# JakobHavtorn/benchmarking-lvms

Hardware: AMD Instinct MI355X
Metric: audio frames/sec training (VRNN, 16 kHz mu-law) (higher is better)
Workload: dtype f32

## Files before the change

benchmarking-lvms_amd/csrc/core.hip:

```cpp
#include <stdarg.h>
#include <string.h>

#include <stdlib.h>

#include <mutex>

#include "common.h"

namespace blvm {

static thread_local char g_err[512] = "";

void set_error(const char* fmt, ...) {
  va_list ap;
  va_start(ap, fmt);
  vsnprintf(g_err, sizeof(g_err), fmt, ap);
  va_end(ap);
}

}

namespace blvm {
namespace {
struct I32Chunk { int32_t v[256]; };
__global__ __launch_bounds__(256) void upload_i32_kernel(I32Chunk c, int32_t* dst, int n) {
  if ((int)threadIdx.x < n) dst[threadIdx.x] = c.v[threadIdx.x];
}
}
}

extern "C" int blvm_upload_i32(const int32_t* host, int n, int32_t* dst, void* stream) {
  using namespace blvm;
  BLVM_REQUIRE(n >= 0 && (n == 0 || (host != nullptr && dst != nullptr)), "upload_i32: null pointer");
  for (int off = 0; off < n; off += 256) {
    I32Chunk c;
    const int m = n - off < 256 ? n - off : 256;
    memcpy(c.v, host + off, sizeof(int32_t) * m);
    hipLaunchKernelGGL(upload_i32_kernel, dim3(1), dim3(256), 0, static_cast<hipStream_t>(stream), c, dst + off, m);
  }
  BLVM_CHECK_LAUNCH("upload_i32");
  return BLVM_OK;
}

namespace blvm {
namespace {
struct PchainCtl {
  std::mutex mu;
  int device = -1;
  unsigned* dev = nullptr;
  unsigned* host = nullptr;
  unsigned* host_dev = nullptr;
  unsigned epoch = 0;
  unsigned taken = 0;
};
PchainCtl& pchain_ctl_state() {
  static PchainCtl c;
  return c;
}
}

namespace {
int g_pchain_max_b = -1, g_pchain_tune = -1;
unsigned long long* g_pchain_prof = nullptr;
}
unsigned long long* pchain_profile_buffer() { return g_pchain_prof; }
int pchain_max_batch() {
  if (g_pchain_max_b < 0) {
    const char* e = getenv("BLVM_PCHAIN");
    const char* m = getenv("BLVM_PCHAIN_MAX_B");
    g_pchain_max_b = (e && atoi(e) == 0) ? 0 : (m ? atoi(m) : 128);
    for (const char* v : {"HSA_CU_MASK", "ROC_GLOBAL_CU_MASK"})
      if (const char* cm = getenv(v); cm && *cm) g_pchain_max_b = 0;
  }
  return g_pchain_max_b;
}
static_assert(OP_F32 == BLVM_DTYPE_F32 && OP_BF16 == BLVM_DTYPE_BF16 && OP_F16 == BLVM_DTYPE_F16, "operand types are the ABI values");
static int g_operand_dtype = -1;
OpType operand_type() {
  if (g_operand_dtype < 0) {
    const char* e = getenv("BLVM_DTYPE");
    g_operand_dtype = !e ? OP_F32
                      : (strcmp(e, "bf16") == 0 || strcmp(e, "1") == 0) ? OP_BF16
                      : (strcmp(e, "f16") == 0 || strcmp(e, "2") == 0)  ? OP_F16
                                                                          : OP_F32;
  }
  return static_cast<OpType>(g_operand_dtype);
}
int pchain_tune() {
  if (g_pchain_tune < 0) {
    const char* e = getenv("BLVM_PCHAIN_TUNE");
    g_pchain_tune = e ? atoi(e) : 20;
  }
  return g_pchain_tune;
}

int pchain_ctl(unsigned** dev, unsigned** host_dev, unsigned* epoch) {
  PchainCtl& c = pchain_ctl_state();
  std::lock_guard<std::mutex> lock(c.mu);
  int d = 0;
  BLVM_HIP(hipGetDevice(&d));
  if (c.device != d) {
    BLVM_HIP(hipMalloc(reinterpret_cast<void**>(&c.dev), 64));
    BLVM_HIP(hipMemset(c.dev, 0, 64));
    BLVM_HIP(hipHostMalloc(reinterpret_cast<void**>(&c.host), 64, hipHostMallocMapped));
    memset(c.host, 0, 64);
    BLVM_HIP(hipHostGetDevicePointer(reinterpret_cast<void**>(&c.host_dev), c.host, 0));
    c.device = d;
    c.epoch = 0;
    c.taken = 0;
  }
  *dev = c.dev;
  *host_dev = c.host_dev;
  *epoch = ++c.epoch;
  if (c.epoch == 0) *epoch = ++c.epoch;
  return BLVM_OK;
}
}

extern "C" int blvm_pchain_configure(int max_batch, int waves) {
  if (waves > 0 && waves != 16) {
    blvm::set_error("blvm_pchain_configure: waves = %d; the persistent kernels run 16 waves per workgroup", waves);
    return BLVM_EINVAL;
  }
  if (max_batch >= 0) blvm::g_pchain_max_b = max_batch;
  return BLVM_OK;
}

extern "C" int blvm_set_operand_dtype(int dtype) {
  if (dtype != BLVM_DTYPE_F32 && dtype != BLVM_DTYPE_BF16 && dtype != BLVM_DTYPE_F16) {
    blvm::set_error("blvm_set_operand_dtype: %d is none of BLVM_DTYPE_F32 (0), BLVM_DTYPE_BF16 (1), BLVM_DTYPE_F16 (2)", dtype);
    return BLVM_EINVAL;
  }
  blvm::g_operand_dtype = dtype;
  return BLVM_OK;
}
extern "C" int blvm_get_operand_dtype(void) { return blvm::operand_type(); }

extern "C" int blvm_pchain_max_batch(void) { return std::min(blvm::pchain_max_batch(), 128); }

extern "C" int blvm_pchain_tune(int bits) {
  blvm::g_pchain_tune = bits;
  return BLVM_OK;
}

extern "C" int blvm_pchain_profile(unsigned long long* device_buffer) {
  blvm::g_pchain_prof = device_buffer;
  return BLVM_OK;
}

extern "C" int blvm_async_errors(unsigned* last_code) {
  blvm::PchainCtl& c = blvm::pchain_ctl_state();
  std::lock_guard<std::mutex> lock(c.mu);
  if (!c.host) return 0;
  const volatile unsigned* h = c.host;
  if (last_code) *last_code = h[1];
  return (int)h[0];
}

extern "C" int blvm_async_errors_take(unsigned* last_code) {
  blvm::PchainCtl& c = blvm::pchain_ctl_state();
  std::lock_guard<std::mutex> lock(c.mu);
  if (!c.host) return 0;
  const volatile unsigned* h = c.host;
  const unsigned total = h[0];
  const unsigned fresh = total - c.taken;
  c.taken = total;
  if (last_code) *last_code = fresh ? h[1] : 0u;
  return (int)fresh;
}

extern "C" int blvm_version(void) { return 130;  }

extern "C" const char* blvm_last_error(void) { return blvm::g_err; }

// ... 13 lines not shown
```

benchmarking-lvms_amd/csrc/vrnn_static.h:

```cpp
#pragma once
#include <algorithm>
#include <initializer_list>

#include "pchain.h"

namespace blvm {
namespace pchain {

struct LinkRange {
  int ct, wg0, nwg;
};
struct VrnnFwdDeal {
  int def_n, half, g;
  LinkRange hproj, prior, post, head, phi, gru;
};
inline VrnnFwdDeal vrnn_fwd_deal(int ctH, int ctZ, int ctR, int tl, int cus, bool shared) {
  VrnnFwdDeal d;
  d.def_n = shared ? 0 : range_for(3 * ctR * tl, std::min(cus / 4, 64));
  d.half = range_for(ctH * tl, (cus - d.def_n) / 2);
  d.g = 2 * d.half;
  const int wide = shared ? d.half : d.g;
  d.hproj = shared ? LinkRange{3 * ctR, d.half, d.half} : LinkRange{3 * ctR, d.g, d.def_n};
  d.prior = LinkRange{ctH, 0, d.half};
  d.post = LinkRange{ctH, d.half, d.half};
  d.head = LinkRange{ctZ, 0, range_for(ctZ * tl, wide)};
  d.phi = LinkRange{ctH, 0, range_for(ctH * tl, wide)};
  d.gru = LinkRange{ctR, 0, range_for(ctR * tl, d.g)};
  return d;
}
struct VrnnBwdDeal {
  int def_n, half, g, spare;
  bool split3;
  LinkRange grub, part[3], dphi, gb, wide_h, dz, prior, post;
};
inline VrnnBwdDeal vrnn_bwd_deal(int ctH, int ctZ, int ctR, int tl, int cus, bool shared, bool allow_split3) {
  VrnnBwdDeal d;
  d.def_n = shared ? 0 : range_for(ctR * tl, std::min(cus / 4, 64));
  d.half = range_for(ctH * tl, (cus - d.def_n) / 2);
  d.g = 2 * d.half;
  const int wide = shared ? d.half : d.g;
  d.spare = cus - d.g - d.def_n;
  d.split3 = !shared && d.spare >= 8 && d.half >= 8 && allow_split3;
  d.grub = LinkRange{ctR, 0, range_for(ctR * tl, d.g)};
  d.part[0] = LinkRange{ctH, 0, range_for(ctH * tl, d.half)};
  d.part[1] = LinkRange{ctH, d.half, range_for(ctH * tl, d.half)};
  d.part[2] = LinkRange{ctH, d.g + d.def_n, d.split3 ? range_for(ctH * tl, d.spare) : 0};
  d.dphi = LinkRange{ctH, 0, range_for(ctH * tl, wide)};
  d.gb = shared ? LinkRange{ctR, d.half, d.half} : LinkRange{ctR, d.g, d.def_n};
  d.wide_h = LinkRange{ctH, 0, range_for(ctH * tl, wide)};
  d.dz = LinkRange{ctZ, 0, range_for(ctZ * tl, wide)};
  d.prior = LinkRange{ctH, 0, d.half};
  d.post = LinkRange{ctH, d.half, d.half};
  return d;
}

constexpr std::initializer_list<int> kFwdResident = {1, 2, 3, 4, 5};
constexpr std::initializer_list<int> kBwdResident = {0, 1, 2, 3, 5, 6, 7, 8, 9};
inline bool one_tile_each(const Program& p, std::initializer_list<int> links) {
  for (int i : links)
    if (tiles_per_workgroup((p.B + 15) / 16, p.d[i].ct, p.d[i].nwg, p.xcd != 0) > 1) return false;
  return true;
}

}
}
```

benchmarking-lvms_amd/csrc/vrnn_static.hip:

```cpp
#include <algorithm>
#include <mutex>

#include "common.h"
#include "pchain.h"
#include "vrnn_static.h"

namespace blvm {
namespace {
using namespace pchain;

struct SPtr {
  float* base;
  int stride;
  __device__ __forceinline__ float* at(int s) const { return base + (long)s * stride; }
};

constexpr int kMaxTiles = 8;
__device__ __forceinline__ int tile_lanes(int w, int wg0, int nwg, int rt, int ct, bool xcd) {
  TileIter it(w, wg0, nwg, rt, ct, xcd);
  const int lane = threadIdx.x & 63;
  it.j += lane * it.step;
  return (lane < kMaxTiles && it.valid()) ? (it.r0() | (it.c() << 16)) : -1;
}
__device__ __forceinline__ int tile_count(int lanes) { return __popcll(__ballot(lanes >= 0)); }

constexpr int kAnatBase = 128, kAnatRole = 512, kAnatSlots = 48;
#ifdef PCHAIN_TPROF
__device__ __forceinline__ void anat_begin(unsigned* tab) {
  for (int i = threadIdx.x; i < kAnatSlots * 8; i += blockDim.x) tab[i] = 0u;
  __syncthreads();
}
__device__ __forceinline__ void anat_arm(Poll& pl) { pl.rpolls = 0; pl.t_st = 0; }
__device__ __forceinline__ void anat_note(unsigned* tab, int slot, const Poll& pl) {
  const unsigned long long now = wall_clock64();
  if ((threadIdx.x & 63) == 0 && pl.rpolls != 0) {
    unsigned* q = tab + (slot * 2 + (threadIdx.x < 256 ? 0 : 1)) * 4;
    atomicAdd(q, 1u); atomicAdd(q + 1, pl.rpolls); atomicAdd(q + 2, (unsigned)(pl.t_ok - pl.t_issue));
    atomicAdd(q + 3, (unsigned)((pl.t_st != 0 ? pl.t_st : now) - pl.t_ok));
  }
}
__device__ __forceinline__ void anat_end(const unsigned* tab, unsigned long long* prof, int role, bool chosen) {
  __syncthreads();
  if (prof != nullptr && chosen)
    for (int i = threadIdx.x; i < kAnatSlots * 8; i += blockDim.x) prof[kAnatBase + role * kAnatRole + i] = tab[i];
}
#define ANAT(x) x
#else
#define ANAT(x)
#endif

struct LinChainArgs {
  SPtr a16, orm, o16;
  const float *W, *bias;
  int ldo, n16, B, s0, S, wg0, nwg, ct, xcd;
  Ctl ctl;
  int pace_early, pace_epi;
  ANAT(unsigned long long* prof;)
};
template <class PC>
__device__ __forceinline__ PC chain_pace(const LinChainArgs& a) {
  if constexpr (PC::paced) return PC{a.pace_early, a.pace_epi};
  else return PC();
}

template <int NW, int K, bool RES, class PC = PaceOff>
__global__ __launch_bounds__(NW * 64, 1) void static_lin_chain_kernel(LinChainArgs a) {
  __shared__ __attribute__((aligned(16))) float red[2][NW * 256];
  ANAT(__shared__ unsigned anat[kAnatSlots * 8]; anat_begin(anat);)
  const int w = blockIdx.x, B = a.B;
  const int tiles = tile_lanes(w, a.wg0, a.nwg, (B + 15) / 16, a.ct, a.xcd != 0);
  const int nt = tile_count(tiles);
  if (nt == 0) return;
  Poll pl{a.ctl, 0u, false, 1};
  int par = 0;
  if constexpr (RES) {
    const int trc = __builtin_amdgcn_readlane(tiles, 0), r0 = trc & 0xffff, c0 = (trc >> 16) * 16;
    WRegs<OP_F32, 1, K / (16 * NW)> ws;
    const float* const Ws[1] = {a.W};
    const int cs[1] = {c0};
    load_w<NW, OP_F32, 1, K / (16 * NW)>(ws.w, Ws, cs, K);
    const PC pace = chain_pace<PC>(a);
    for (int s = a.s0; s < a.S; ++s) {
      pl.code = (unsigned)s << 4;
      auto late = [&]() { return LinLate{a.bias, nullptr, nullptr, 0, 0, false, true, 0.f, Out{a.orm.at(s), a.ldo, false, a.o16.at(s), a.n16}}; };
      ANAT(anat_arm(pl);)
      tile_lin_late<NW, OP_F32>(a.a16.at(s), 0, true, a.W, K, late, r0, c0, B, red[par], pl, nullptr, nullptr, 0, ws, pace);
      ANAT(anat_note(anat, 0, pl);)
      par ^= 1;
    }
    ANAT(anat_end(anat, a.prof, 0, w == a.wg0);)
    return;
  }
  for (int s = a.s0; s < a.S; ++s) {
    pl.code = (unsigned)s << 4;
    const float* A = a.a16.at(s);
    auto late = [&]() { return LinLate{a.bias, nullptr, nullptr, 0, 0, false, true, 0.f, Out{a.orm.at(s), a.ldo, false, a.o16.at(s), a.n16}}; };
    for (int tk = 0; tk < nt; ++tk) {
      const int trc = __builtin_amdgcn_readlane(tiles, tk);
      tile_lin_late<NW, false>(A, 0, true, a.W, K, late, trc & 0xffff, (trc >> 16) * 16, B, red[par], pl);
      par ^= 1;
    }
  }
}

constexpr int kH = 256, kR = 512;

struct LinArgs {
  SPtr a, a2, a3, add, gate, orm, o16, o16b;
  const float *W, *bias;
  int ld0, ld1, ld2, ld3, n16, n16b, w_width;
  float slope;
};
struct SeqArgs {
  SPtr a0, add0, aux[4], orm[4], o16[4];
  const float* W[4];
  int ld[4], ldadd0, ldgate, n16;
  float slope;
};
struct HeadArgs {
  SPtr P, Q, eps, mu_p, sd_p, mu_q, sd_q, raw_p, raw_q, muq_raw, z, z16, z16b;
  const float *Wp, *bp, *Wq, *bq;
  int ld3, n16, n16b, Z, residual;
  float beta, inv_beta, sd_eps;
};
struct GruArgs {
  SPtr X, xg, gh, hprev, hrm, h16, h16b, rg, ug, ng;
  const float *Wih, *bih;
  int ld0, ld3, n16, n16b, R;
};
struct DzArgs {
  SPtr D, add, mu_q, sd_q, mu_p, sd_p, eps, raw_q, raw_p, muq_raw, dqh, dqh16, dph, dph16;
  const float *WT, *c_raw, *c_fn;
  const int32_t* x_sl;
  int ld1, ld3, n16, Z, residual, stride, t0, first_gemm;
  float fn_floor, beta, sd_eps;
};
struct GrubArgs {
  SPtr D0, D1, g_in, rg, ug, ng, gh, hprev, dd, dgi, dgi16, dgh, dgh16, ga, g_add;
  const float *W0, *W1, *g_out;
  int ld0, ld1, ld3, n16, R, first_gemm, end_gates, first_gin;
};
struct Deal {
  int wg0, nwg, ct, s_begin, s_end, idx;
};

struct Walk {
  float* red0;
  float* red1;
  int par, B;
  Poll pl;
  ANAT(unsigned* anat;)
  __device__ __forceinline__ float* red() { par ^= 1; return par ? red0 : red1; }
  __device__ __forceinline__ void at(const Deal& d, int s, bool gentle, unsigned li = 0) {
// ... 95 lines not shown
    if (li == 0) tile_lin_late<NW, OP_F32>(A, 0, true, q.W[li], K0, late, tr0, tc0, wk.B, wk.red(), wk.pl, nullptr, nullptr, 0, rr.first, P0());
    else tile_lin_late<NW, OP_F32>(A, 0, true, q.W[li], K, late, tr0, tc0, wk.B, wk.red(), wk.pl, nullptr, nullptr, 0, rr.rest[li > 0 ? li - 1 : 0], Paced());
    ANAT(anat_note(wk.anat, 4 * d.idx + li, wk.pl);)
    A = q.o16[li].at(s);
  }
}

template <int NW, class PC = PaceOff>
__device__ __forceinline__ void visit_head(const HeadArgs& q, const Deal& d, int s, int tiles, int nt, Walk& wk, const Res<kH, 4>& ws) {
  if (nt == 0 || s < d.s_begin || s >= d.s_end) return;
  wk.at(d, s, false);
  const HeadOut o{q.mu_p.at(s), q.sd_p.at(s), q.mu_q.at(s), q.sd_q.at(s), q.raw_p.at(s), q.raw_q.at(s), q.muq_raw.at(s),
                  Out{q.z.at(s), q.ld3, false, q.z16.at(s), q.n16, q.z16b.at(s), q.n16b}};
  const int trc = __builtin_amdgcn_readlane(tiles, 0);
  ANAT(anat_arm(wk.pl);)
  tile_head<NW, OP_F32>(q.P.at(s), q.Q.at(s), true, q.Wp, q.bp, q.Wq, q.bq, q.eps.at(s), o, kH, q.Z, q.residual, q.beta, q.inv_beta, q.sd_eps,
                        trc & 0xffff, (trc >> 16) * 16, wk.B, wk.red(), wk.pl, ws, PC());
  ANAT(anat_note(wk.anat, 4 * d.idx, wk.pl);)
}

template <int NW, class PC = PaceOff>
__device__ __forceinline__ void visit_gru(const GruArgs& q, const Deal& d, int s, int tiles, int nt, Walk& wk, const Res<kH, 3>& ws) {
  if (nt == 0 || s < d.s_begin || s >= d.s_end) return;
  wk.at(d, s, false);
  const Out o{q.hrm.at(s), q.ld3, true, q.h16.at(s), q.n16, q.h16b.at(s), q.n16b};
  const int trc = __builtin_amdgcn_readlane(tiles, 0);
  ANAT(anat_arm(wk.pl);)
  tile_gru<NW, OP_F32>(q.X.at(s), 0, true, q.Wih, kH, q.xg.at(s), q.bih, q.gh.at(s), q.hprev.at(s), q.ld0, q.R, o, q.rg.at(s), q.ug.at(s), q.ng.at(s),
                       trc & 0xffff, (trc >> 16) * 16, wk.B, wk.red(), wk.pl, ws, PC());
  ANAT(anat_note(wk.anat, 4 * d.idx, wk.pl);)
}

template <int NW, class PC = PaceOff>
__device__ __forceinline__ void visit_dz(const DzArgs& q, const Deal& d, int s, int tiles, int nt, Walk& wk, const Res<kH>& ws) {
  if (nt == 0 || s < d.s_begin || s >= d.s_end) return;
  wk.at(d, s, false);
  DzIn z;
  z.mu_q = q.mu_q.at(s); z.sd_q = q.sd_q.at(s); z.mu_p = q.mu_p.at(s); z.sd_p = q.sd_p.at(s); z.eps = q.eps.at(s); z.raw_q = q.raw_q.at(s);
  z.raw_p = q.raw_p.at(s); z.muq_raw = q.muq_raw.at(s);
  z.x_sl = q.x_sl; z.c_raw = q.c_raw; z.c_fn = q.c_fn;
  z.t = q.t0 - s; z.stride = q.stride; z.residual = q.residual;
  z.fn_floor = q.fn_floor; z.beta = q.beta; z.sd_eps = q.sd_eps;
  z.has_gemm = s >= q.first_gemm;
  const Out oq{q.dqh.at(s), q.ld3, false, q.dqh16.at(s), q.n16}, op{q.dph.at(s), q.ld3, false, q.dph16.at(s), q.n16};
  const int trc = __builtin_amdgcn_readlane(tiles, 0);
  ANAT(anat_arm(wk.pl);)
  tile_dz<NW, OP_F32>(q.D.at(s), q.WT, nullptr, nullptr, true, q.add.at(s), q.ld1, false, z, oq, op, kH, q.Z, trc & 0xffff, (trc >> 16) * 16, wk.B,
                      wk.red(), wk.pl, ws, PC());
  ANAT(anat_note(wk.anat, 4 * d.idx, wk.pl);)
}

template <int NW, class PC = PaceOff>
__device__ __forceinline__ void visit_grub(const GrubArgs& q, const Deal& d, int s, int tiles, int nt, Walk& wk, const Res<kH, 2>& ws) {
  if (nt == 0 || s < d.s_begin || s >= d.s_end) return;
  wk.at(d, s, false);
  GrubIn g;
  g.D0 = q.D0.at(s); g.D1 = q.D1.at(s); g.W0 = q.W0; g.W1 = q.W1; g.g_in = q.g_in.at(s); g.g_add = q.g_add.at(s); g.ld_gadd = q.ld1;
  g.rg = q.rg.at(s); g.ug = q.ug.at(s); g.ng = q.ng.at(s); g.gh = q.gh.at(s); g.hprev = q.hprev.at(s); g.dd = q.dd.at(s); g.ldh = q.ld0;
  g.dgi = Out{q.dgi.at(s), q.ld3, false, q.dgi16.at(s), q.n16};
  g.dgh = Out{q.dgh.at(s), q.ld3, false, q.dgh16.at(s), q.n16};
  g.ga = q.ga.at(s); g.g_out = const_cast<float*>(q.g_out);
  g.has_gemm = s >= q.first_gemm; g.has_gates = s < q.end_gates; g.has_gin = s >= q.first_gin;
  const int trc = __builtin_amdgcn_readlane(tiles, 0);
  ANAT(anat_arm(wk.pl);)
  tile_grub<NW, OP_F32>(g, kH, q.R, trc & 0xffff, (trc >> 16) * 16, wk.B, wk.red(), wk.pl, ws, PC());
  ANAT(anat_note(wk.anat, 4 * d.idx, wk.pl);)
}

template <class A>
__device__ __forceinline__ const A& kargs() {
  typedef const __attribute__((address_space(4))) char kchar;
  kchar* p = (kchar*)__builtin_amdgcn_kernarg_segment_ptr();
  asm volatile("" : "+s"(p));
  return *(const A*)p;
}

struct FwdArgs {
  LinArgs hproj;
  SeqArgs run[2];
  HeadArgs head;
  SeqArgs phi;
  GruArgs gru;
  Deal deal[6];
  int B, s0, S, xcd;
  Ctl ctl;
  ANAT(unsigned long long* prof;)
};
constexpr int kFwdProducts = 4, kBwdProducts = 2;

template <int NW, int HALF>
__device__ __forceinline__ void fwd_half(const FwdArgs& a, int w, int rt, bool xcd, Walk& wk) {
  const int t1 = tile_lanes(w, a.deal[1 + HALF].wg0, a.deal[1 + HALF].nwg, rt, a.deal[1 + HALF].ct, xcd), n1 = tile_count(t1);
  const int t3 = tile_lanes(w, a.deal[3].wg0, a.deal[3].nwg, rt, a.deal[3].ct, xcd), n3 = tile_count(t3);
  const int t4 = tile_lanes(w, a.deal[4].wg0, a.deal[4].nwg, rt, a.deal[4].ct, xcd), n4 = tile_count(t4);
  const int t5 = tile_lanes(w, a.deal[5].wg0, a.deal[5].nwg, rt, a.deal[5].ct, xcd), n5 = tile_count(t5);
  RunRes<3, kR, kH> run;
  Res<kH, 4> head;
  RunRes<4, kH, kH> phi;
  Res<kH, 3> gru;
  load_run<NW>(run, kargs<FwdArgs>().run[HALF], t1, n1);
  load_head<NW>(head, kargs<FwdArgs>().head, t3, n3);
  load_run<NW>(phi, kargs<FwdArgs>().phi, t4, n4);
  load_gru<NW>(gru, kargs<FwdArgs>().gru, t5, n5);
  for (int s = a.s0; s < a.S; ++s) {
    visit_run<NW, 3, kR, kH, false, Paced>(kargs<FwdArgs>().run[HALF], kargs<FwdArgs>().deal[1 + HALF], s, t1, n1, wk, run);
    visit_head<NW, Paced>(kargs<FwdArgs>().head, kargs<FwdArgs>().deal[3], s, t3, n3, wk, head);
    visit_run<NW, 4, kH, kH, false, Paced>(kargs<FwdArgs>().phi, kargs<FwdArgs>().deal[4], s, t4, n4, wk, phi);
    if constexpr (HALF == 0) visit_gru<NW, Paced>(kargs<FwdArgs>().gru, kargs<FwdArgs>().deal[5], s, t5, n5, wk, gru);
    else visit_gru<NW>(kargs<FwdArgs>().gru, kargs<FwdArgs>().deal[5], s, t5, n5, wk, gru);
  }
  ANAT(anat_end(wk.anat, kargs<FwdArgs>().prof, HALF, w == kargs<FwdArgs>().deal[1 + HALF].wg0);)
}

template <int NW>
__global__ __launch_bounds__(NW * 64, 1) void vrnn_static_fwd_kernel(FwdArgs a) {
  extern __shared__ __attribute__((aligned(16))) float lds_red[];
  const int w = blockIdx.x, rt = (a.B + 15) / 16;
  const bool xcd = a.xcd != 0;
  Walk wk{lds_red, lds_red + kFwdProducts * NW * 256, 0, a.B, Poll{a.ctl, 0u, false, 1}};
  ANAT(__shared__ unsigned anat[kAnatSlots * 8]; anat_begin(anat); wk.anat = anat;)
  if (w >= a.deal[0].wg0) {
    const int t0 = tile_lanes(w, a.deal[0].wg0, a.deal[0].nwg, rt, a.deal[0].ct, xcd), n0 = tile_count(t0);
    if (n0 == 0) return;
    for (int s = a.s0; s < a.S; ++s) visit_lin<NW, kR, DF_RM_SC1 | DF_GENTLE | DF_CANARY>(kargs<FwdArgs>().hproj, kargs<FwdArgs>().deal[0], s, t0, n0, wk, WMem());
    return;
  }
  if (w < a.deal[2].wg0) fwd_half<NW, 0>(a, w, rt, xcd, wk);
  else fwd_half<NW, 1>(a, w, rt, xcd, wk);
}

struct BwdArgs {
  GrubArgs grub;
  LinArgs part[3], gb, sum;
  SeqArgs phi;
  DzArgs dz;
  SeqArgs run[2];
  Deal deal[10];
  int B, s0, S, xcd;
  Ctl ctl;
  ANAT(unsigned long long* prof;)
};

template <int NW, int HALF>
__device__ __forceinline__ void bwd_half(const BwdArgs& a, int w, int rt, bool xcd, Walk& wk) {
  const int t0 = tile_lanes(w, a.deal[0].wg0, a.deal[0].nwg, rt, a.deal[0].ct, xcd), n0 = tile_count(t0);
  const int t1 = tile_lanes(w, a.deal[1 + HALF].wg0, a.deal[1 + HALF].nwg, rt, a.deal[1 + HALF].ct, xcd), n1 = tile_count(t1);
  const int t5 = tile_lanes(w, a.deal[5].wg0, a.deal[5].nwg, rt, a.deal[5].ct, xcd), n5 = tile_count(t5);
  const int t6 = tile_lanes(w, a.deal[6].wg0, a.deal[6].nwg, rt, a.deal[6].ct, xcd), n6 = tile_count(t6);
  const int t7 = tile_lanes(w, a.deal[7].wg0, a.deal[7].nwg, rt, a.deal[7].ct, xcd), n7 = tile_count(t7);
  const int t8 = tile_lanes(w, a.deal[8 + HALF].wg0, a.deal[8 + HALF].nwg, rt, a.deal[8 + HALF].ct, xcd), n8 = tile_count(t8);
  Res<kH, 2> grub;
  Res<kR> part;
  Res<kH> sum, dz;
  RunRes<2, kH, kH> phi;
  RunRes<3, 2 * kH, kH> run;
  load_grub<NW>(grub, kargs<BwdArgs>().grub, t0, n0);
  load_lin<NW, kR>(part, kargs<BwdArgs>().part[HALF].W, kargs<BwdArgs>().part[HALF].w_width, t1, n1);
  load_lin<NW, kH>(sum, kargs<BwdArgs>().sum.W, kH, t5, n5);
  load_run<NW>(phi, kargs<BwdArgs>().phi, t6, n6);
  load_lin<NW, kH>(dz, kargs<BwdArgs>().dz.WT, kH, t7, n7);
  load_run<NW>(run, kargs<BwdArgs>().run[HALF], t8, n8);
  for (int s = a.s0; s < a.S; ++s) {
    visit_grub<NW, Paced>(kargs<BwdArgs>().grub, kargs<BwdArgs>().deal[0], s, t0, n0, wk, grub);
    visit_lin<NW, kR, 0, Paced>(kargs<BwdArgs>().part[HALF], kargs<BwdArgs>().deal[1 + HALF], s, t1, n1, wk, part);
    visit_lin<NW, kH, DF_A_SUM3, Paced>(kargs<BwdArgs>().sum, kargs<BwdArgs>().deal[5], s, t5, n5, wk, sum);
    visit_run<NW, 2, kH, kH, true, Paced>(kargs<BwdArgs>().phi, kargs<BwdArgs>().deal[6], s, t6, n6, wk, phi);
    visit_dz<NW, Paced>(kargs<BwdArgs>().dz, kargs<BwdArgs>().deal[7], s, t7, n7, wk, dz);
    if constexpr (HALF == 0) visit_run<NW, 3, 2 * kH, kH, true, Paced>(kargs<BwdArgs>().run[HALF], kargs<BwdArgs>().deal[8 + HALF], s, t8, n8, wk, run);
    else visit_run<NW, 3, 2 * kH, kH, true>(kargs<BwdArgs>().run[HALF], kargs<BwdArgs>().deal[8 + HALF], s, t8, n8, wk, run);
  }
  ANAT(anat_end(wk.anat, kargs<BwdArgs>().prof, 2 + HALF, w == kargs<BwdArgs>().deal[1 + HALF].wg0);)
}

template <int NW>
__global__ __launch_bounds__(NW * 64, 1) void vrnn_static_bwd_kernel(BwdArgs a) {
  extern __shared__ __attribute__((aligned(16))) float lds_red[];
  const int w = blockIdx.x, rt = (a.B + 15) / 16;
  const bool xcd = a.xcd != 0;
  Walk wk{lds_red, lds_red + kBwdProducts * NW * 256, 0, a.B, Poll{a.ctl, 0u, false, 1}};
  ANAT(__shared__ unsigned anat[kAnatSlots * 8]; anat_begin(anat); wk.anat = anat;)
  if (w >= a.deal[3].wg0) {
    const int t = tile_lanes(w, a.deal[3].wg0, a.deal[3].nwg, rt, a.deal[3].ct, xcd), n = tile_count(t);
    if (n == 0) return;
    Res<kR> part;
    load_lin<NW, kR>(part, kargs<BwdArgs>().part[2].W, kargs<BwdArgs>().part[2].w_width, t, n);
    for (int s = a.s0; s < a.S; ++s) visit_lin<NW, kR, 0>(kargs<BwdArgs>().part[2], kargs<BwdArgs>().deal[3], s, t, n, wk, part);
    ANAT(anat_end(wk.anat, kargs<BwdArgs>().prof, 4, w == kargs<BwdArgs>().deal[3].wg0);)
    return;
  }
  if (w >= a.deal[4].wg0) {
    const int t = tile_lanes(w, a.deal[4].wg0, a.deal[4].nwg, rt, a.deal[4].ct, xcd), n = tile_count(t);
    if (n == 0) return;
    for (int s = a.s0; s < a.S; ++s)
      visit_lin<NW, 3 * kR, DF_ADD_POLLED | DF_RM_SC1 | DF_GENTLE | DF_CANARY>(kargs<BwdArgs>().gb, kargs<BwdArgs>().deal[4], s, t, n, wk, WMem());
    return;
  }
  if (w < a.deal[2].wg0) bwd_half<NW, 0>(a, w, rt, xcd, wk);
  else bwd_half<NW, 1>(a, w, rt, xcd, wk);
}

bool int_strides(const Program& p) {
  for (long v : p.stride)
    if (v < -2147483647L || v > 2147483647L) return false;
  return true;
}
SPtr sptr(const Program& p, const Desc& d, int k) { return SPtr{const_cast<float*>(d.p[k]), (int)p.stride[d.sidx[k]]}; }

template <class Kern>
int static_go(Kern kernel, int slot, int grid, size_t lds, const char* what) {
  static std::mutex mu;
  static int attr_dev[3] = {-1, -1, -1}, occ[3] = {0, 0, 0};
  int dev = 0, cus = 0;
  BLVM_HIP(hipGetDevice(&dev));
  BLVM_HIP(hipDeviceGetAttribute(&cus, hipDeviceAttributeMultiprocessorCount, dev));
  {
    std::lock_guard<std::mutex> lock(mu);
    if (attr_dev[slot] != dev) {
      BLVM_HIP(hipFuncSetAttribute(reinterpret_cast<const void*>(kernel), hipFuncAttributeMaxDynamicSharedMemorySize, (int)lds));
      BLVM_HIP(hipOccupancyMaxActiveBlocksPerMultiprocessor(&occ[slot], kernel, 1024, lds));
      attr_dev[slot] = dev;
    }
    BLVM_REQUIRE((long)occ[slot] * cus >= grid, "%s: %d workgroups are not co-resident (%d per CU x %d CUs)", what, grid, occ[slot], cus);
  }
  return BLVM_OK;
}

int static_lin_chain_launch(const Program& p, hipStream_t stream, bool resident, bool pace = false, int early = 0, int epi = 0) {
  if (p.ndesc != 1 || p.ot != OP_F32 || p.rt_group != 1 || !int_strides(p)) return 1;
  const Desc& d = p.d[0];
  if (d.kind != K_LIN || d.flags != DF_RELU || d.f[LIN_F_SLOPE] != 0.f || (d.K != 256 && d.K != 512) || d.s_begin != 0 || d.s_end != p.S) return 1;
  if (d.ld[LIN_LD_A] != 0 || d.i[LIN_I_W_WIDTH] != 0 || d.p[LIN_ADD] || d.p[LIN_GATE] || d.p[LIN_O16B] || d.p[LIN_A2] || d.p[LIN_A3] || d.n16[N16_OUTB] != 0)
    return 1;
  const int rt = (p.B + 15) / 16;
  if (d.nwg <= 0 || (p.xcd && d.nwg % 8 != 0) || tiles_per_workgroup(rt, d.ct, d.nwg, p.xcd != 0) > (resident ? 1 : kMaxTiles)) return 1;
  LinChainArgs a{sptr(p, d, LIN_A), sptr(p, d, LIN_ORM), sptr(p, d, LIN_O16), d.p[LIN_W], d.p[LIN_BIAS], d.ld[LD_OUT], d.n16[N16_OUT], p.B, p.s_first, p.S,
                 d.wg0, d.nwg, d.ct, p.xcd, p.ctl, early, epi};
  ANAT(a.prof = pchain_profile_buffer();)
  const int grid = d.wg0 + d.nwg;
  auto go = [&](auto kernel) -> int {
    BLVM_TRY(static_go(kernel, 2, grid, 0, "static_lin_chain"));
    hipLaunchKernelGGL(kernel, dim3(grid), dim3(1024), 0, stream, a);
    BLVM_CHECK_LAUNCH("static_lin_chain");
    return BLVM_OK;
  };
  if (resident && pace) return d.K == 256 ? go(&static_lin_chain_kernel<16, 256, true, PaceRt>) : go(&static_lin_chain_kernel<16, 512, true, PaceRt>);
  if (resident) return d.K == 256 ? go(&static_lin_chain_kernel<16, 256, true>) : go(&static_lin_chain_kernel<16, 512, true>);
  return d.K == 256 ? go(&static_lin_chain_kernel<16, 256, false>) : go(&static_lin_chain_kernel<16, 512, false>);
}

int g_static = 1;
long g_static_launches = 0;
bool pchain_static_on() { return g_static != 0; }

SPtr sp(const Program& p, const Desc& d, int k) { return SPtr{const_cast<float*>(d.p[k]), d.p[k] ? (int)p.stride[d.sidx[k]] : 0}; }
Deal deal_of(const Desc& d, int idx) { return Deal{d.wg0, d.nwg, d.ct, d.s_begin, d.s_end, idx}; }
bool within(const Desc& d, int lo, int hi) { return d.wg0 >= lo && d.wg0 + d.nwg <= hi; }
bool few_tiles(const Program& p, const Desc& d) {
  if (d.nwg <= 0 || (p.xcd && d.nwg % 8 != 0)) return false;
  return tiles_per_workgroup((p.B + 15) / 16, d.ct, d.nwg, p.xcd != 0) <= kMaxTiles;
}
bool shaped(const Desc& d, int kind, int flags, int K) { return d.kind == kind && d.flags == flags && d.K == K; }
bool run(const Desc& d, int n, int K0) { return d.i[LINSEQ_I_N] == n && d.i[LINSEQ_I_K0] == K0; }

LinArgs lin_args(const Program& p, const Desc& d) {
  return LinArgs{sp(p, d, LIN_A), sp(p, d, LIN_A2), sp(p, d, LIN_A3), sp(p, d, LIN_ADD), sp(p, d, LIN_GATE), sp(p, d, LIN_ORM), sp(p, d, LIN_O16),
                 sp(p, d, LIN_O16B), d.p[LIN_W], d.p[LIN_BIAS], d.ld[LIN_LD_A], d.ld[LIN_LD_ADD], d.ld[LIN_LD_GATE], d.ld[LD_OUT], d.n16[N16_OUT], d.n16[N16_OUTB],
                 d.i[LIN_I_W_WIDTH], d.f[LIN_F_SLOPE]};
}
SeqArgs seq_args(const Program& p, const Desc& d) {
  SeqArgs q{};
  q.a0 = sp(p, d, LINSEQ_A0); q.add0 = sp(p, d, LINSEQ_ADD0);
  for (int i = 0; i < d.i[LINSEQ_I_N]; ++i) {
    q.W[i] = d.p[LINSEQ_W + i]; q.aux[i] = sp(p, d, LINSEQ_AUX + i); q.orm[i] = sp(p, d, LINSEQ_ORM + i); q.o16[i] = sp(p, d, LINSEQ_O16 + i);
    q.ld[i] = d.ld[LINSEQ_LD_ORM + i];
  }
  q.ldadd0 = d.i[LINSEQ_I_LD_ADD0]; q.ldgate = d.i[LINSEQ_I_LD_GATE]; q.n16 = d.n16[N16_OUT]; q.slope = d.f[LINSEQ_F_SLOPE];
  return q;
}

int vrnn_static_check(const Program& p, int ndesc, int products) {
  if (!pchain_static_on() || p.ndesc != ndesc || p.ot != OP_F32 || p.rt_group != 1 || p.s_first != 0 || p.B > 64) return 1;
  if (p.lds_products != products || !int_strides(p)) return 1;
  for (int i = 0; i < p.ndesc; ++i)
    if (!few_tiles(p, p.d[i])) return 1;
  return 0;
}

int vrnn_static_fwd(const Program& p, hipStream_t stream) {
  if (vrnn_static_check(p, 6, kFwdProducts)) return 1;
  const Desc* d = p.d;
  const int S = p.S;
  for (int i = 0; i < 6; ++i)
    if (d[i].s_begin != 0 || d[i].s_end != S) return 1;
  if (!shaped(d[0], K_LIN, DF_RM_SC1 | DF_GENTLE | DF_CANARY, kR) || !shaped(d[1], K_LINSEQ, DF_RELU, kH) || !shaped(d[2], K_LINSEQ, DF_RELU, kH) ||
      !shaped(d[3], K_HEAD, 0, kH) || !shaped(d[4], K_LINSEQ, DF_RELU, kH) || !shaped(d[5], K_GRU, 0, kH))
    return 1;
  if (!run(d[1], 3, kR) || !run(d[2], 3, kR) || !run(d[4], 4, 0)) return 1;
  if (!one_tile_each(p, kFwdResident)) return 1;
  const int half = d[2].wg0, gentle = d[0].wg0;
  if (d[1].wg0 != 0 || !within(d[1], 0, half) || !within(d[2], half, gentle) || d[0].nwg <= 0) return 1;
  for (int i = 3; i < 6; ++i)
    if (!within(d[i], 0, gentle)) return 1;
  FwdArgs a{};
  a.hproj = lin_args(p, d[0]);
  a.run[0] = seq_args(p, d[1]); a.run[1] = seq_args(p, d[2]); a.phi = seq_args(p, d[4]);
  const Desc &h = d[3], &g = d[5];
  a.head = HeadArgs{sp(p, h, HEAD_P16), sp(p, h, HEAD_Q16), sp(p, h, HEAD_EPS), sp(p, h, HEAD_MU_P), sp(p, h, HEAD_SD_P), sp(p, h, HEAD_MU_Q),
                    sp(p, h, HEAD_SD_Q), sp(p, h, HEAD_RAW_P), sp(p, h, HEAD_RAW_Q), sp(p, h, HEAD_MUQ_RAW), sp(p, h, HEAD_Z), sp(p, h, HEAD_Z16),
                    sp(p, h, HEAD_Z16B), h.p[HEAD_WP], h.p[HEAD_BP], h.p[HEAD_WQ], h.p[HEAD_BQ], h.ld[LD_OUT], h.n16[N16_OUT], h.n16[N16_OUTB],
                    h.i[HEAD_I_Z], h.i[HEAD_I_RESIDUAL], h.f[HEAD_F_BETA], h.f[HEAD_F_INV_BETA], h.f[HEAD_F_SD_EPS]};
  a.gru = GruArgs{sp(p, g, GRU_X16), sp(p, g, GRU_XG), sp(p, g, GRU_GH), sp(p, g, GRU_HPREV), sp(p, g, GRU_HRM), sp(p, g, GRU_H16), sp(p, g, GRU_H16B),
                  sp(p, g, GRU_RG), sp(p, g, GRU_UG), sp(p, g, GRU_NG), g.p[GRU_WIH], g.p[GRU_BIH], g.ld[GRU_LD_HPREV], g.ld[LD_OUT], g.n16[N16_OUT],
                  g.n16[N16_OUTB], g.i[GRU_I_R]};
  int grid = 0;
  for (int i = 0; i < 6; ++i) { a.deal[i] = deal_of(d[i], i); grid = std::max(grid, d[i].wg0 + d[i].nwg); }
  a.B = p.B; a.s0 = p.s_first; a.S = S; a.xcd = p.xcd; a.ctl = p.ctl;
  ANAT(a.prof = pchain_profile_buffer();)
  const size_t lds = sizeof(float) * 2 * kFwdProducts * 16 * 256;
  BLVM_TRY(static_go(&vrnn_static_fwd_kernel<16>, 0, grid, lds, "vrnn_static_fwd"));
  hipLaunchKernelGGL(vrnn_static_fwd_kernel<16>, dim3(grid), dim3(1024), lds, stream, a);
  BLVM_CHECK_LAUNCH("vrnn_static_fwd");
  ++g_static_launches;
  return BLVM_OK;
}

int vrnn_static_bwd(const Program& p, hipStream_t stream) {
  if (vrnn_static_check(p, 10, kBwdProducts)) return 1;
  const Desc* d = p.d;
  const int S = p.S;
  for (int i = 0; i < 10; ++i)
    if (d[i].s_begin != 0 || d[i].s_end != (i == 0 ? S : S - 1)) return 1;
  if (!shaped(d[0], K_GRUB, 0, kH) || !shaped(d[1], K_LIN, 0, kR) || !shaped(d[2], K_LIN, 0, kR) || !shaped(d[3], K_LIN, 0, kR) ||
      !shaped(d[4], K_LIN, DF_ADD_POLLED | DF_RM_SC1 | DF_GENTLE | DF_CANARY, 3 * kR) || !shaped(d[5], K_LIN, DF_A_SUM3, kH) ||
      !shaped(d[6], K_LINSEQ, DF_SEQ_GATE, kH) || !shaped(d[7], K_DZ, 0, kH) || !shaped(d[8], K_LINSEQ, DF_SEQ_GATE, kH) ||
      !shaped(d[9], K_LINSEQ, DF_SEQ_GATE, kH))
    return 1;
  if (!run(d[6], 2, 0) || !run(d[8], 3, 2 * kH) || !run(d[9], 3, 2 * kH)) return 1;
  if (!one_tile_each(p, kBwdResident) || d[7].p[DZ_D2_16] != nullptr) return 1;
  const int half = d[2].wg0, gentle = d[4].wg0, spare = d[3].wg0;
  if (!within(d[1], 0, half) || !within(d[8], 0, half) || !within(d[2], half, gentle) || !within(d[9], half, gentle) || !within(d[4], gentle, spare) ||
      d[3].nwg <= 0)
    return 1;
  for (int i : {0, 5, 6, 7})
    if (!within(d[i], 0, gentle)) return 1;
  BwdArgs a{};
  const Desc& g = d[0];
  a.grub = GrubArgs{sp(p, g, GRUB_D0_16), sp(p, g, GRUB_D1_16), sp(p, g, GRUB_G_IN), sp(p, g, GRUB_RG), sp(p, g, GRUB_UG), sp(p, g, GRUB_NG), sp(p, g, GRUB_GH),
                    sp(p, g, GRUB_HPREV), sp(p, g, GRUB_DD), sp(p, g, GRUB_DGI), sp(p, g, GRUB_DGI16), sp(p, g, GRUB_DGH), sp(p, g, GRUB_DGH16), sp(p, g, GRUB_GA),
                    sp(p, g, GRUB_G_ADD), g.p[GRUB_W0], g.p[GRUB_W1], g.p[GRUB_G_OUT], g.ld[GRUB_LD_H], g.ld[GRUB_LD_GADD], g.ld[LD_OUT], g.n16[N16_OUT],
                    g.i[GRUB_I_R], g.i[GRUB_I_GEMM_FROM], g.i[GRUB_I_GATES_TO], g.i[GRUB_I_GIN_FROM]};
  for (int k = 0; k < 3; ++k) a.part[k] = lin_args(p, d[1 + k]);
  a.gb = lin_args(p, d[4]); a.sum = lin_args(p, d[5]);
  a.phi = seq_args(p, d[6]); a.run[0] = seq_args(p, d[8]); a.run[1] = seq_args(p, d[9]);
  const Desc& z = d[7];
  a.dz = DzArgs{sp(p, z, DZ_D16), sp(p, z, DZ_ADD), sp(p, z, DZ_MU_Q), sp(p, z, DZ_SD_Q), sp(p, z, DZ_MU_P), sp(p, z, DZ_SD_P),
                sp(p, z, DZ_EPS), sp(p, z, DZ_RAW_Q), sp(p, z, DZ_RAW_P), sp(p, z, DZ_MUQ_RAW), sp(p, z, DZ_DQH), sp(p, z, DZ_DQH16), sp(p, z, DZ_DPH),
                sp(p, z, DZ_DPH16), z.p[DZ_WT], z.p[DZ_C_RAW], z.p[DZ_C_FN], reinterpret_cast<const int32_t*>(z.p[DZ_X_SL]), z.ld[DZ_LD_ADD],
                z.ld[LD_OUT], z.n16[N16_OUT], z.i[DZ_I_Z], z.i[DZ_I_RESIDUAL], z.i[DZ_I_STRIDE], z.i[DZ_I_T0], (int)z.f[DZ_F_GEMM_FROM], z.f[DZ_F_FN_FLOOR],
                z.f[DZ_F_BETA], z.f[DZ_F_SD_EPS]};
  int grid = 0;
  for (int i = 0; i < 10; ++i) { a.deal[i] = deal_of(d[i], i); grid = std::max(grid, d[i].wg0 + d[i].nwg); }
  a.B = p.B; a.s0 = p.s_first; a.S = S; a.xcd = p.xcd; a.ctl = p.ctl;
  ANAT(a.prof = pchain_profile_buffer();)
  const size_t lds = sizeof(float) * 2 * kBwdProducts * 16 * 256;
  BLVM_TRY(static_go(&vrnn_static_bwd_kernel<16>, 1, grid, lds, "vrnn_static_bwd"));
  hipLaunchKernelGGL(vrnn_static_bwd_kernel<16>, dim3(grid), dim3(1024), lds, stream, a);
  BLVM_CHECK_LAUNCH("vrnn_static_bwd");
  ++g_static_launches;
  return BLVM_OK;
}

}

int vrnn_launch(pchain::Builder& bld, bool forward, const char* who, hipStream_t stream) {
  BLVM_TRY(pchain_prepare(bld, who));
  const int rc = forward ? vrnn_static_fwd(bld.p, stream) : vrnn_static_bwd(bld.p, stream);
  return rc == 1 ? pchain_run(bld.p, stream) : rc;
}

}

extern "C" int blvm_pchain_static(int mode) {
  if (mode == -2) return (int)std::min<long>(blvm::g_static_launches, 0x7fffffffL);
  const int was = blvm::g_static;
  if (mode >= 0) blvm::g_static = mode != 0;
  return was;
}

static int static_chain_probe(const float* W16, const float* bias, float* x16, float* xs, int B, int N, int L, int nwg, void* stream_, bool resident,
                              bool pace = false, int early = 0, int epi = 0) {
  using namespace blvm;
  using namespace blvm::pchain;
  hipStream_t s = static_cast<hipStream_t>(stream_);
  BLVM_REQUIRE(W16 && bias && x16 && xs && B > 0 && N > 0 && N % 16 == 0 && L > 0, "pchain_static_chain_probe: bad arguments");
  const int rt = (B + 15) / 16;
  const long x = (long)rt * 16 * N, sN = (long)B * N;
  Builder bld;
  bld.begin(OP_F32, L, B, 1, false, 0);
  const int nw = nwg > 0 ? nwg : range_for((N / 16) * rt, device_cus() & ~7);
  Operands o;
  o.p[LIN_A] = {x16, x}; o.p[LIN_W] = W16; o.p[LIN_BIAS] = bias; o.p[LIN_ORM] = {xs, sN}; o.p[LIN_O16] = {x16 + x, x}; o.ld[LD_OUT] = N; o.n16[N16_OUT] = N / 16;
  add_desc(bld, K_LIN, N / 16, 0, nw, N, DF_RELU, 0, L, o);
  BLVM_HIP(pchain_fill_sentinel(x16 + x, sizeof(float) * (size_t)x * L, s));
  BLVM_TRY(pchain_prepare(bld, "pchain_static_chain_probe"));
  const int rc = static_lin_chain_launch(bld.p, s, resident, pace, early, epi);
  BLVM_REQUIRE(rc != 1, "pchain_static_chain_probe: no static kernel for N = %d (256, 512) or this deal", N);
  return rc;
}
extern "C" int blvm_pchain_static_chain_probe(const float* W16, const float* bias, float* x16, float* xs, int B, int N, int L, int nwg, void* stream) {
  return static_chain_probe(W16, bias, x16, xs, B, N, L, nwg, stream, true);
}
extern "C" int blvm_pchain_static_chain_probe_fetch(const float* W16, const float* bias, float* x16, float* xs, int B, int N, int L, int nwg, void* stream) {
  return static_chain_probe(W16, bias, x16, xs, B, N, L, nwg, stream, false);
}
extern "C" int blvm_pchain_static_chain_probe_paced(const float* W16, const float* bias, float* x16, float* xs, int B, int N, int L, int nwg,
                                                    int early_delay, int epi_delay, void* stream) {
  using namespace blvm;
  BLVM_REQUIRE(early_delay >= 0 && early_delay <= 64 && epi_delay >= 0 && epi_delay <= 64,
               "pchain_static_chain_probe_paced: delays are 0 .. 64 s_sleep units");
  return static_chain_probe(W16, bias, x16, xs, B, N, L, nwg, stream, true, (early_delay | epi_delay) != 0, early_delay, epi_delay);
}
```

Baseline: 85.45 million.

## Add XCD-local workgroup placement for persistent VRNN kernels and enable by default

Adds a workgroup placement mode that remaps blockIdx so that for a batch of 4 row tiles the prior/post halves land on chosen XCD groups (place_wg interleaving), bypassing the program's own xcd-aware tile iteration. The default tune bits change from 20 to 84, which sets bit 64 so local placement is requested when the deal layout qualifies and falls back otherwise. The intent is to keep communicating workgroups on the same XCD, cutting cross-die L2 traffic and polling latency in the persistent chain kernels. The risk is worse load balance, or behaviour changes when the layout check rejects the configuration.

```diff
diff --git a/benchmarking-lvms_amd/csrc/core.hip b/benchmarking-lvms_amd/csrc/core.hip
--- a/benchmarking-lvms_amd/csrc/core.hip
+++ b/benchmarking-lvms_amd/csrc/core.hip
@@ -89,7 +89,7 @@
 int pchain_tune() {
   if (g_pchain_tune < 0) {
     const char* e = getenv("BLVM_PCHAIN_TUNE");
-    g_pchain_tune = e ? atoi(e) : 20;
+    g_pchain_tune = e ? atoi(e) : 84;
   }
   return g_pchain_tune;
 }
diff --git a/benchmarking-lvms_amd/csrc/vrnn_static.h b/benchmarking-lvms_amd/csrc/vrnn_static.h
--- a/benchmarking-lvms_amd/csrc/vrnn_static.h
+++ b/benchmarking-lvms_amd/csrc/vrnn_static.h
@@ -56,10 +56,39 @@
 
 constexpr std::initializer_list<int> kFwdResident = {1, 2, 3, 4, 5};
 constexpr std::initializer_list<int> kBwdResident = {0, 1, 2, 3, 5, 6, 7, 8, 9};
-inline bool one_tile_each(const Program& p, std::initializer_list<int> links) {
+inline bool one_tile_each(const Program& p, std::initializer_list<int> links, bool xcd) {
   for (int i : links)
-    if (tiles_per_workgroup((p.B + 15) / 16, p.d[i].ct, p.d[i].nwg, p.xcd != 0) > 1) return false;
+    if (tiles_per_workgroup((p.B + 15) / 16, p.d[i].ct, p.d[i].nwg, xcd) > 1) return false;
   return true;
+}
+inline bool one_tile_each(const Program& p, std::initializer_list<int> links) { return one_tile_each(p, links, p.xcd != 0); }
+
+enum Place {
+  kPlaceProgram = 0,
+  kPlacePlain = 1,
+  kPlaceLocal = 2,
+};
+constexpr int kPlaceSpan = 128;
+__host__ __device__ __forceinline__ int place_wg(int p) { return p < kPlaceSpan ? 64 * ((p & 7) >> 2) + 4 * (p >> 3) + (p & 3) : p; }
+inline bool place_local_applies(const Program& p, int prior, int post, int grid) {
+  if ((p.B + 15) / 16 != 4 || grid < kPlaceSpan) return false;
+  if (p.d[prior].wg0 != 0 || p.d[prior].nwg != 64 || p.d[post].wg0 != 64 || p.d[post].nwg != 64) return false;
+  for (int i = 0; i < p.ndesc; ++i) {
+    const int lo = p.d[i].wg0, hi = lo + p.d[i].nwg;
+    const bool kept = (lo == 0 && (hi == 64 || hi == kPlaceSpan)) || (lo == 64 && hi == kPlaceSpan) || lo >= kPlaceSpan;
+    if (!kept) return false;
+  }
+  return true;
+}
+inline int place_for(int want, int fallback, const Program& p, int prior, int post, int grid) {
+  if (want == kPlaceLocal) return place_local_applies(p, prior, post, grid) ? kPlaceLocal : (fallback == kPlacePlain ? kPlacePlain : kPlaceProgram);
+  return want == kPlacePlain ? kPlacePlain : kPlaceProgram;
+}
+inline bool place_xcd(int place, const Program& p) { return place == kPlaceProgram && p.xcd != 0; }
+inline int grid_of(const Program& p) {
+  int g = 0;
+  for (int i = 0; i < p.ndesc; ++i) g = std::max(g, p.d[i].wg0 + p.d[i].nwg);
+  return g;
 }
 
 }
diff --git a/benchmarking-lvms_amd/csrc/vrnn_static.hip b/benchmarking-lvms_amd/csrc/vrnn_static.hip
--- a/benchmarking-lvms_amd/csrc/vrnn_static.hip
+++ b/benchmarking-lvms_amd/csrc/vrnn_static.hip
@@ -16,6 +16,7 @@
 };
 
 constexpr int kMaxTiles = 8;
+__device__ __forceinline__ int placed_wg(int place) { return place == kPlaceLocal ? place_wg((int)blockIdx.x) : (int)blockIdx.x; }
 __device__ __forceinline__ int tile_lanes(int w, int wg0, int nwg, int rt, int ct, bool xcd) {
   TileIter it(w, wg0, nwg, rt, ct, xcd);
   const int lane = threadIdx.x & 63;
@@ -52,7 +53,7 @@
 struct LinChainArgs {
   SPtr a16, orm, o16;
   const float *W, *bias;
-  int ldo, n16, B, s0, S, wg0, nwg, ct, xcd;
+  int ldo, n16, B, s0, S, wg0, nwg, ct, xcd, place;
   Ctl ctl;
   int pace_early, pace_epi;
   ANAT(unsigned long long* prof;)
@@ -67,8 +68,8 @@
 __global__ __launch_bounds__(NW * 64, 1) void static_lin_chain_kernel(LinChainArgs a) {
   __shared__ __attribute__((aligned(16))) float red[2][NW * 256];
   ANAT(__shared__ unsigned anat[kAnatSlots * 8]; anat_begin(anat);)
-  const int w = blockIdx.x, B = a.B;
-  const int tiles = tile_lanes(w, a.wg0, a.nwg, (B + 15) / 16, a.ct, a.xcd != 0);
+  const int w = placed_wg(a.place), B = a.B;
+  const int tiles = tile_lanes(w, a.wg0, a.nwg, (B + 15) / 16, a.ct, a.place == kPlaceProgram && a.xcd != 0);
   const int nt = tile_count(tiles);
   if (nt == 0) return;
   Poll pl{a.ctl, 0u, false, 1};
@@ -330,7 +331,7 @@
   SeqArgs phi;
   GruArgs gru;
   Deal deal[6];
-  int B, s0, S, xcd;
+  int B, s0, S, xcd, place;
   Ctl ctl;
   ANAT(unsigned long long* prof;)
 };
@@ -363,8 +364,8 @@
 template <int NW>
 __global__ __launch_bounds__(NW * 64, 1) void vrnn_static_fwd_kernel(FwdArgs a) {
   extern __shared__ __attribute__((aligned(16))) float lds_red[];
-  const int w = blockIdx.x, rt = (a.B + 15) / 16;
-  const bool xcd = a.xcd != 0;
+  const int w = placed_wg(a.place), rt = (a.B + 15) / 16;
+  const bool xcd = a.place == kPlaceProgram && a.xcd != 0;
   Walk wk{lds_red, lds_red + kFwdProducts * NW * 256, 0, a.B, Poll{a.ctl, 0u, false, 1}};
   ANAT(__shared__ unsigned anat[kAnatSlots * 8]; anat_begin(anat); wk.anat = anat;)
   if (w >= a.deal[0].wg0) {
@@ -384,7 +385,7 @@
   DzArgs dz;
   SeqArgs run[2];
   Deal deal[10];
-  int B, s0, S, xcd;
+  int B, s0, S, xcd, place;
   Ctl ctl;
   ANAT(unsigned long long* prof;)
 };
@@ -423,8 +424,8 @@
 template <int NW>
 __global__ __launch_bounds__(NW * 64, 1) void vrnn_static_bwd_kernel(BwdArgs a) {
   extern __shared__ __attribute__((aligned(16))) float lds_red[];
-  const int w = blockIdx.x, rt = (a.B + 15) / 16;
-  const bool xcd = a.xcd != 0;
+  const int w = placed_wg(a.place), rt = (a.B + 15) / 16;
+  const bool xcd = a.place == kPlaceProgram && a.xcd != 0;
   Walk wk{lds_red, lds_red + kBwdProducts * NW * 256, 0, a.B, Poll{a.ctl, 0u, false, 1}};
   ANAT(__shared__ unsigned anat[kAnatSlots * 8]; anat_begin(anat); wk.anat = anat;)
   if (w >= a.deal[3].wg0) {
@@ -446,6 +447,9 @@
   if (w < a.deal[2].wg0) bwd_half<NW, 0>(a, w, rt, xcd, wk);
   else bwd_half<NW, 1>(a, w, rt, xcd, wk);
 }
+
+int static_place_fallback() { return (pchain_tune() & 32) ? kPlacePlain : kPlaceProgram; }
+int static_place_wanted() { return (pchain_tune() & 64) ? kPlaceLocal : static_place_fallback(); }
 
 bool int_strides(const Program& p) {
   for (long v : p.stride)
@@ -480,11 +484,14 @@
   if (d.ld[LIN_LD_A] != 0 || d.i[LIN_I_W_WIDTH] != 0 || d.p[LIN_ADD] || d.p[LIN_GATE] || d.p[LIN_O16B] || d.p[LIN_A2] || d.p[LIN_A3] || d.n16[N16_OUTB] != 0)
     return 1;
   const int rt = (p.B + 15) / 16;
-  if (d.nwg <= 0 || (p.xcd && d.nwg % 8 != 0) || tiles_per_workgroup(rt, d.ct, d.nwg, p.xcd != 0) > (resident ? 1 : kMaxTiles)) return 1;
+  int place = resident ? static_place_wanted() : kPlaceProgram;
+  if (place == kPlaceLocal && !(rt == 4 && d.wg0 == 0 && (d.nwg == 64 || d.nwg == kPlaceSpan) && device_cus() >= kPlaceSpan)) place = static_place_fallback();
+  const bool xcd = place == kPlaceProgram && p.xcd != 0;
+  if (d.nwg <= 0 || (p.xcd && d.nwg % 8 != 0) || tiles_per_workgroup(rt, d.ct, d.nwg, xcd) > (resident ? 1 : kMaxTiles)) return 1;
   LinChainArgs a{sptr(p, d, LIN_A), sptr(p, d, LIN_ORM), sptr(p, d, LIN_O16), d.p[LIN_W], d.p[LIN_BIAS], d.ld[LD_OUT], d.n16[N16_OUT], p.B, p.s_first, p.S,
-                 d.wg0, d.nwg, d.ct, p.xcd, p.ctl, early, epi};
+                 d.wg0, d.nwg, d.ct, p.xcd, place, p.ctl, early, epi};
   ANAT(a.prof = pchain_profile_buffer();)
-  const int grid = d.wg0 + d.nwg;
+  const int grid = place == kPlaceLocal ? kPlaceSpan : d.wg0 + d.nwg;
   auto go = [&](auto kernel) -> int {
     BLVM_TRY(static_go(kernel, 2, grid, 0, "static_lin_chain"));
     hipLaunchKernelGGL(kernel, dim3(grid), dim3(1024), 0, stream, a);
@@ -503,9 +510,9 @@
 SPtr sp(const Program& p, const Desc& d, int k) { return SPtr{const_cast<float*>(d.p[k]), d.p[k] ? (int)p.stride[d.sidx[k]] : 0}; }
 Deal deal_of(const Desc& d, int idx) { return Deal{d.wg0, d.nwg, d.ct, d.s_begin, d.s_end, idx}; }
 bool within(const Desc& d, int lo, int hi) { return d.wg0 >= lo && d.wg0 + d.nwg <= hi; }
-bool few_tiles(const Program& p, const Desc& d) {
+bool few_tiles(const Program& p, const Desc& d, bool xcd) {
   if (d.nwg <= 0 || (p.xcd && d.nwg % 8 != 0)) return false;
-  return tiles_per_workgroup((p.B + 15) / 16, d.ct, d.nwg, p.xcd != 0) <= kMaxTiles;
+  return tiles_per_workgroup((p.B + 15) / 16, d.ct, d.nwg, xcd) <= kMaxTiles;
 }
 bool shaped(const Desc& d, int kind, int flags, int K) { return d.kind == kind && d.flags == flags && d.K == K; }
 bool run(const Desc& d, int n, int K0) { return d.i[LINSEQ_I_N] == n && d.i[LINSEQ_I_K0] == K0; }
@@ -526,16 +533,18 @@
   return q;
 }
 
-int vrnn_static_check(const Program& p, int ndesc, int products) {
+int vrnn_static_check(const Program& p, int ndesc, int products, int prior, int post, int* place) {
   if (!pchain_static_on() || p.ndesc != ndesc || p.ot != OP_F32 || p.rt_group != 1 || p.s_first != 0 || p.B > 64) return 1;
   if (p.lds_products != products || !int_strides(p)) return 1;
+  *place = place_for(static_place_wanted(), static_place_fallback(), p, prior, post, grid_of(p));
   for (int i = 0; i < p.ndesc; ++i)
-    if (!few_tiles(p, p.d[i])) return 1;
+    if (!few_tiles(p, p.d[i], place_xcd(*place, p))) return 1;
   return 0;
 }
 
 int vrnn_static_fwd(const Program& p, hipStream_t stream) {
-  if (vrnn_static_check(p, 6, kFwdProducts)) return 1;
+  int place = kPlaceProgram;
+  if (vrnn_static_check(p, 6, kFwdProducts, 1, 2, &place)) return 1;
   const Desc* d = p.d;
   const int S = p.S;
   for (int i = 0; i < 6; ++i)
@@ -544,7 +553,7 @@
       !shaped(d[3], K_HEAD, 0, kH) || !shaped(d[4], K_LINSEQ, DF_RELU, kH) || !shaped(d[5], K_GRU, 0, kH))
     return 1;
   if (!run(d[1], 3, kR) || !run(d[2], 3, kR) || !run(d[4], 4, 0)) return 1;
-  if (!one_tile_each(p, kFwdResident)) return 1;
+  if (!one_tile_each(p, kFwdResident, place_xcd(place, p))) return 1;
   const int half = d[2].wg0, gentle = d[0].wg0;
   if (d[1].wg0 != 0 || !within(d[1], 0, half) || !within(d[2], half, gentle) || d[0].nwg <= 0) return 1;
   for (int i = 3; i < 6; ++i)
@@ -562,7 +571,7 @@
                   g.n16[N16_OUTB], g.i[GRU_I_R]};
   int grid = 0;
   for (int i = 0; i < 6; ++i) { a.deal[i] = deal_of(d[i], i); grid = std::max(grid, d[i].wg0 + d[i].nwg); }
-  a.B = p.B; a.s0 = p.s_first; a.S = S; a.xcd = p.xcd; a.ctl = p.ctl;
+  a.B = p.B; a.s0 = p.s_first; a.S = S; a.xcd = p.xcd; a.place = place; a.ctl = p.ctl;
   ANAT(a.prof = pchain_profile_buffer();)
   const size_t lds = sizeof(float) * 2 * kFwdProducts * 16 * 256;
   BLVM_TRY(static_go(&vrnn_static_fwd_kernel<16>, 0, grid, lds, "vrnn_static_fwd"));
@@ -573,7 +582,8 @@
 }
 
 int vrnn_static_bwd(const Program& p, hipStream_t stream) {
-  if (vrnn_static_check(p, 10, kBwdProducts)) return 1;
+  int place = kPlaceProgram;
+  if (vrnn_static_check(p, 10, kBwdProducts, 8, 9, &place)) return 1;
   const Desc* d = p.d;
   const int S = p.S;
   for (int i = 0; i < 10; ++i)
@@ -584,7 +594,7 @@
       !shaped(d[9], K_LINSEQ, DF_SEQ_GATE, kH))
     return 1;
   if (!run(d[6], 2, 0) || !run(d[8], 3, 2 * kH) || !run(d[9], 3, 2 * kH)) return 1;
-  if (!one_tile_each(p, kBwdResident) || d[7].p[DZ_D2_16] != nullptr) return 1;
+  if (!one_tile_each(p, kBwdResident, place_xcd(place, p)) || d[7].p[DZ_D2_16] != nullptr) return 1;
   const int half = d[2].wg0, gentle = d[4].wg0, spare = d[3].wg0;
   if (!within(d[1], 0, half) || !within(d[8], 0, half) || !within(d[2], half, gentle) || !within(d[9], half, gentle) || !within(d[4], gentle, spare) ||
       d[3].nwg <= 0)
@@ -608,7 +618,7 @@
                 z.f[DZ_F_BETA], z.f[DZ_F_SD_EPS]};
   int grid = 0;
   for (int i = 0; i < 10; ++i) { a.deal[i] = deal_of(d[i], i); grid = std::max(grid, d[i].wg0 + d[i].nwg); }
-  a.B = p.B; a.s0 = p.s_first; a.S = S; a.xcd = p.xcd; a.ctl = p.ctl;
+  a.B = p.B; a.s0 = p.s_first; a.S = S; a.xcd = p.xcd; a.place = place; a.ctl = p.ctl;
   ANAT(a.prof = pchain_profile_buffer();)
   const size_t lds = sizeof(float) * 2 * kBwdProducts * 16 * 256;
   BLVM_TRY(static_go(&vrnn_static_bwd_kernel<16>, 1, grid, lds, "vrnn_static_bwd"));
```

Result: faster. 87.80 million (median of 6 runs) (+2.7%).
